# daxmawal/StarPU-Inference-Server

Measured on AMD Instinct MI355X. Metric: inferences/sec + p50 latency, ResNet-18 bs=1 & BERT-base seq=128, 1/2/4/8 GPU, higher is better.
Workload: dtype fp16m; 1 GPU; ResNet-18 bs=8 fp16, single MI355X HIP codelet (conv-as-implicit-GEMM MFMA); batch_per_task=8, workers_per_gpu=4, parallelism=replicas x1 (request sharding, no collective)

## Files before the change

starpu-inference-server_amd/csrc/conv_wres.hip:

```cpp
#include "lds_dma.hpp"
#include "spi_kernels.hpp"

#include <algorithm>
#include <cstdlib>
#include <stdexcept>
#include <type_traits>

namespace spi {
namespace {

constexpr int kRowB = 128;
constexpr int kWImg = 64 * kRowB;
constexpr int kWBytes = 9 * kWImg;
constexpr int kHaloPix = 256;
constexpr int kHBuf = kHaloPix * kRowB;
constexpr int kLds = kHBuf + kWBytes;
constexpr int BM = 128, BN = 64, NT = 256;
constexpr int kWPieces = kWBytes / 1024 / 4;
constexpr int kHPieces = kHBuf / 1024 / 4;

struct WresArgs {
  const _Float16* x;
  const char* w;
  const float* bias;
  const _Float16* res;
  _Float16* y;
  const char* zeros;
  int H, W;
  int th;
  int bands_per_img, bands;
};

#ifdef SPI_WRES_STAMPS
__device__ unsigned long long g_wres_stamps[4096 * 10];
#define WRES_STAMP(k)                                                                   \
  do {                                                                                  \
    __builtin_amdgcn_sched_barrier(0);                                                  \
    if (tid == 0 && blockIdx.x < 4096) g_wres_stamps[blockIdx.x * 10 + (k)] = __builtin_amdgcn_s_memtime(); \
    __builtin_amdgcn_sched_barrier(0);                                                  \
  } while (0)
#else
#define WRES_STAMP(k) \
  do {                \
  } while (0)
#endif

template <bool HAS_RES, bool RELU>
__global__ __launch_bounds__(NT, 1) void conv3x3_c64_wres(WresArgs a) {
  constexpr int kW0 = kHBuf;
  __shared__ __attribute__((aligned(16))) char lds[kLds];
  const int tid = threadIdx.x, lane = tid & 63, wave = __builtin_amdgcn_readfirstlane(tid >> 6);
  int wg = blockIdx.x;
  {
    const int nwg = gridDim.x, q = nwg >> 3, r = nwg & 7, x = wg & 7, l = wg >> 3;
    if (nwg >= 16) wg = (x < r ? x * (q + 1) : r * (q + 1) + (x - r) * q) + l;
  }
  const int band = wg;
  if (band >= a.bands) return;
  const int Wp = a.W + 2;
  const int hp = (a.th + 2) * Wp;
#ifdef SPI_WRES_STAMPS
  if (tid == 0 && blockIdx.x < 4096) g_wres_stamps[blockIdx.x * 10 + 9] = __builtin_amdgcn_s_memrealtime();
#endif
  WRES_STAMP(0);

  const char* wimg = a.w + (size_t)64 * (9 * kRowB);
  auto issue_w = [&] {
#pragma unroll
    for (int i = 0; i < kWPieces; ++i) {
      const int q = i * 4 + wave;
      glds16(wimg + q * 1024 + lane * 16, lds + kW0 + q * 1024);
    }
  };

  int h_hy[kHPieces], h_off[kHPieces];
  bool h_ok[kHPieces];
#pragma unroll
  for (int i = 0; i < kHPieces; ++i) {
    const int p = ((wave * kHPieces + i) << 3) + (lane >> 3);
    const int c = (lane & 7) ^ (p & 7);
    const int hy = p / Wp, hx = p - hy * Wp;
    h_hy[i] = hy;
    h_ok[i] = p < hp && (unsigned)(hx - 1) < (unsigned)a.W;
    h_off[i] = ((hy - 1) * a.W + (hx - 1)) * 64 + c * 8;
  }
  auto issue_halo = [&] {
    const int img = band / a.bands_per_img, oy0 = (band - img * a.bands_per_img) * a.th;
    const _Float16* base = a.x + ((size_t)img * a.H + oy0) * a.W * 64;
    char* dst = lds;
#pragma unroll
    for (int i = 0; i < kHPieces; ++i) {
      const int iy = oy0 - 1 + h_hy[i];
      const bool ok = h_ok[i] && (unsigned)iy < (unsigned)a.H;
      const char* src = ok ? reinterpret_cast<const char*>(base + h_off[i]) : a.zeros;
      glds16(src, dst + (wave * kHPieces + i) * 1024);
    }
  };

  const int fr = lane & 15, fq = lane >> 4, wm = wave >> 1, wn = wave & 1;
  int aoff[9][2][4];
#pragma unroll
  for (int i = 0; i < 4; ++i) {
    const int r = wm * 64 + i * 16 + fr;
    const int ty = r / a.W, tx = r - ty * a.W;
    const int p0 = ty < a.th ? ty * Wp + tx : 0;
#pragma unroll
    for (int tap = 0; tap < 9; ++tap)
#pragma unroll
      for (int kk = 0; kk < 2; ++kk) {
        const int p = p0 + (tap / 3) * Wp + tap % 3;
        aoff[tap][kk][i] = p * kRowB + (((kk * 4 + fq) ^ (p & 7)) << 4);
      }
  }
  int boff[2][2];
#pragma unroll
  for (int kk = 0; kk < 2; ++kk)
#pragma unroll
    for (int jj = 0; jj < 2; ++jj) {
      const int n = wn * 32 + jj * 16 + fr;
      boff[kk][jj] = kW0 + n * kRowB + (((kk * 4 + fq) ^ (n & 7)) << 4);
    }

  constexpr int E_G = BN / 8, E_RSTEP = NT / E_G, E_ITEMS = BM / E_RSTEP;
  const int e_nb8 = (tid % E_G) * 8, e_r0 = tid / E_G;
  int e_rel[E_ITEMS], e_ty[E_ITEMS];
#pragma unroll
  for (int it = 0; it < E_ITEMS; ++it) {
    const int row = e_r0 + it * E_RSTEP;
    const int ty = row / a.W, tx = row - ty * a.W;
    e_ty[it] = ty < a.th ? ty : 1 << 30;
    e_rel[it] = ty * a.W + tx;
  }

  issue_halo();
  issue_w();
  {
    [[maybe_unused]] constexpr int sk = 1;
    dma_wait_barrier<2 * 8>();
    WRES_STAMP(sk);
    const char* Hs = lds;

    floatx4 acc[4][2];
#pragma unroll
    for (int i = 0; i < 4; ++i)
#pragma unroll
      for (int jj = 0; jj < 2; ++jj) acc[i][jj] = floatx4{0.f, 0.f, 0.f, 0.f};
    half8 fa[2][4], fb[2][2];
    auto load = [&](int t, int s) {
      const int tap = t >> 1, kk = t & 1;
#pragma unroll
      for (int i = 0; i < 4; ++i) fa[s][i] = *reinterpret_cast<const half8*>(Hs + aoff[tap][kk][i]);
#pragma unroll
      for (int jj = 0; jj < 2; ++jj)
        fb[s][jj] = *reinterpret_cast<const half8*>(lds + boff[kk][jj] + tap * kWImg);
    };
    load(0, 0);
    static_for<0, 18>([&](auto tc) {
      constexpr int t = decltype(tc)::value;
      if constexpr (t + 1 < 18) {
        if constexpr ((t + 1) % 2 == 0) {
          constexpr int T = (t + 1) / 2;
          dma_wait_barrier<2 * (8 - T)>();
        }
        load(t + 1, (t + 1) & 1);
      }
      __builtin_amdgcn_sched_barrier(0);
#pragma unroll
      for (int i = 0; i < 4; ++i)
#pragma unroll
        for (int jj = 0; jj < 2; ++jj)
          acc[i][jj] = __builtin_amdgcn_mfma_f32_16x16x32_f16(fa[t & 1][i], fb[t & 1][jj], acc[i][jj], 0, 0, 0);
      __builtin_amdgcn_sched_barrier(0);
    });
    WRES_STAMP(sk + 1);

    const int img = band / a.bands_per_img, oy0 = (band - img * a.bands_per_img) * a.th;
    const int rows_left = a.H - oy0;
    const size_t mbase = ((size_t)img * a.H + oy0) * a.W;
    const floatx4 b0 = *reinterpret_cast<const floatx4*>(a.bias + e_nb8);
    const floatx4 b1 = *reinterpret_cast<const floatx4*>(a.bias + e_nb8 + 4);
    half8 rv[E_ITEMS];
    if constexpr (HAS_RES) {
#pragma unroll
      for (int it = 0; it < E_ITEMS; ++it) {
        const size_t mm = mbase + (e_ty[it] < rows_left ? e_rel[it] : 0);
        rv[it] = *reinterpret_cast<const half8*>(a.res + mm * 64 + e_nb8);
      }
    }
    lds_barrier();
#ifdef SPI_WRES_STAMPS_EPI
    if (sk == 1) WRES_STAMP(4);
#endif
    float* T = reinterpret_cast<float*>(lds);
#pragma unroll
    for (int i = 0; i < 4; ++i)
#pragma unroll
      for (int jj = 0; jj < 2; ++jj)
#pragma unroll
        for (int r = 0; r < 4; ++r) {
          const int row = wm * 64 + i * 16 + fq * 4 + r;
          const int col = (wn * 32 + jj * 16 + fr) ^ (fq << 4);
          T[row * BN + col] = acc[i][jj][r];
        }
#ifdef SPI_WRES_STAMPS_EPI
    if (sk == 1) WRES_STAMP(5);
#endif
    lds_barrier();
#ifdef SPI_WRES_STAMPS_EPI
    if (sk == 1) WRES_STAMP(6);
#endif
    half8 hv[E_ITEMS];
#pragma unroll
    for (int it = 0; it < E_ITEMS; ++it) {
      const int row = e_r0 + it * E_RSTEP;
      const float* src = T + row * BN + (e_nb8 ^ (((row >> 2) & 3) << 4));
      const floatx4 x0 = *reinterpret_cast<const floatx4*>(src);
      const floatx4 x1 = *reinterpret_cast<const floatx4*>(src + 4);
#pragma unroll
      for (int e = 0; e < 8; ++e) {
        float v = (e < 4 ? x0[e] + b0[e] : x1[e - 4] + b1[e - 4]);
        if constexpr (HAS_RES) v += static_cast<float>(rv[it][e]);
        if constexpr (RELU) v = v > 0.f ? v : 0.f;
        hv[it][e] = static_cast<_Float16>(v);
      }
    }
#pragma unroll
    for (int it = 0; it < E_ITEMS; ++it) {
#if defined(SPI_WRES_DIAG) && SPI_WRES_DIAG == 1
      asm volatile("" ::"v"(hv[it]));
#else
      if (e_ty[it] < rows_left) *reinterpret_cast<half8*>(a.y + (mbase + e_rel[it]) * 64 + e_nb8) = hv[it];
#endif
    }
    WRES_STAMP(sk + 2);
  }
  WRES_STAMP(7);
#ifdef SPI_WRES_STAMPS
  if (tid == 0 && blockIdx.x < 4096) g_wres_stamps[blockIdx.x * 10 + 8] = __builtin_amdgcn_s_memrealtime();
#endif
}

int env_int(const char* name, int dflt) {
  const char* e = std::getenv(name);
  return e && *e ? std::atoi(e) : dflt;
}

int& wres_on() {
  static int on = env_int("SPI_CONV_WRES", 1);
  return on;
}

}

void conv_wres_reload_env() { wres_on() = env_int("SPI_CONV_WRES", 1); }

#ifdef SPI_WRES_STAMPS
extern "C" int spi_debug_wres_stamps(unsigned long long* host, size_t n) {
  return hipMemcpyFromSymbol(host, HIP_SYMBOL(g_wres_stamps), n * sizeof(unsigned long long)) == hipSuccess ? 0 : 1;
}
#endif

static int wres_rows(int H, int W) {
  int th = std::min(H, BM / std::max(1, W));
  while (th > 0 && (th + 2) * (W + 2) > kHaloPix) --th;
  return th;
}

constexpr int kWresMaxTiles = 128;

bool conv_wres_eligible(const GemmDesc& d, Prec prec, const GemmPtrs& p) {
  const int on = wres_on();
  if (on == 1 && (d.M + 127) / 128 >= kWresMaxTiles) return false;
  const auto al16 = [](const void* q) { return (reinterpret_cast<uintptr_t>(q) & 15) == 0; };
  return on && prec == Prec::F16 && d.conv && d.KH == 3 && d.KW == 3 && d.stride == 1 && d.pad == 1 &&
         d.Cin == 64 && d.N == 64 && d.K == 576 && d.Kpad == 576 && d.krep == 1 && d.OH == d.H && d.OW == d.W &&
         !d.a_split && !d.out_split && !d.out_f32 && !d.res_f32 && !d.pool_rows && d.ldc == 64 &&
         (!p.res || d.ldr == 64) && d.act != Act::Gelu && wres_rows(d.H, d.W) >= 1 && al16(p.A) && al16(p.W) &&
         al16(p.C) && (!p.res || al16(p.res)) && (!p.bias || al16(p.bias)) && p.zeros && d.w_image;
}

void conv_wres(const GemmDesc& d, const GemmPtrs& p, hipStream_t s) {
  WresArgs a{};
  a.x = static_cast<const _Float16*>(p.A);
  a.w = static_cast<const char*>(p.W);
  a.bias = p.bias ? p.bias : static_cast<const float*>(p.zeros);
  a.res = static_cast<const _Float16*>(p.res);
  a.y = static_cast<_Float16*>(p.C);
  a.zeros = static_cast<const char*>(p.zeros);
  a.H = d.H;
  a.W = d.W;
  a.th = wres_rows(d.H, d.W);
  if (a.th < 1) throw std::invalid_argument("conv_wres: map too wide for the halo buffer");
  a.bands_per_img = (d.H + a.th - 1) / a.th;
  const int imgs = d.M / (d.OH * d.OW);
  a.bands = imgs * a.bands_per_img;
  const bool relu = d.act == Act::Relu;
  const dim3 grid(a.bands);
  if (a.res && relu)
    SPI_LAUNCH((conv3x3_c64_wres<true, true>), grid, dim3(NT), 0, s, a);
  else if (a.res)
    SPI_LAUNCH((conv3x3_c64_wres<true, false>), grid, dim3(NT), 0, s, a);
  else if (relu)
    SPI_LAUNCH((conv3x3_c64_wres<false, true>), grid, dim3(NT), 0, s, a);
  else
    SPI_LAUNCH((conv3x3_c64_wres<false, false>), grid, dim3(NT), 0, s, a);
}

}
```

Baseline: 116,400 inferences/s.

## Keep conv weights in registers per wave and drop weight LDS staging

Each wave now owns 16 output channels and holds its full 3x3x64 weight slice in registers, loaded directly from global memory. The kernel no longer stages weights through LDS, so LDS use shrinks to the halo buffer and launch bounds allow two workgroups per CU. A-operand addressing is computed incrementally, small integer divisions become float-reciprocal multiplies, and MFMA issue is interleaved with LDS reads through sched_group_barrier. This removes weight DMA and B-operand LDS reads. In exchange it costs more VGPRs for 18 weight fragments and 8 accumulators, and each wave now reads A fragments for all 128 rows.

```diff
diff --git a/starpu-inference-server_amd/csrc/conv_wres.hip b/starpu-inference-server_amd/csrc/conv_wres.hip
--- a/starpu-inference-server_amd/csrc/conv_wres.hip
+++ b/starpu-inference-server_amd/csrc/conv_wres.hip
@@ -10,13 +10,12 @@
 namespace {
 
 constexpr int kRowB = 128;
-constexpr int kWImg = 64 * kRowB;
-constexpr int kWBytes = 9 * kWImg;
+constexpr int kWRowB = 9 * kRowB;
 constexpr int kHaloPix = 256;
 constexpr int kHBuf = kHaloPix * kRowB;
-constexpr int kLds = kHBuf + kWBytes;
+constexpr int kLds = kHBuf;
 constexpr int BM = 128, BN = 64, NT = 256;
-constexpr int kWPieces = kWBytes / 1024 / 4;
+constexpr int kChunks = 18;
 constexpr int kHPieces = kHBuf / 1024 / 4;
 
 struct WresArgs {
@@ -46,8 +45,7 @@
 #endif
 
 template <bool HAS_RES, bool RELU>
-__global__ __launch_bounds__(NT, 1) void conv3x3_c64_wres(WresArgs a) {
-  constexpr int kW0 = kHBuf;
+__global__ __launch_bounds__(NT, 2) void conv3x3_c64_wres(WresArgs a) {
   __shared__ __attribute__((aligned(16))) char lds[kLds];
   const int tid = threadIdx.x, lane = tid & 63, wave = __builtin_amdgcn_readfirstlane(tid >> 6);
   int wg = blockIdx.x;
@@ -63,15 +61,8 @@
   if (tid == 0 && blockIdx.x < 4096) g_wres_stamps[blockIdx.x * 10 + 9] = __builtin_amdgcn_s_memrealtime();
 #endif
   WRES_STAMP(0);
-
-  const char* wimg = a.w + (size_t)64 * (9 * kRowB);
-  auto issue_w = [&] {
-#pragma unroll
-    for (int i = 0; i < kWPieces; ++i) {
-      const int q = i * 4 + wave;
-      glds16(wimg + q * 1024 + lane * 16, lds + kW0 + q * 1024);
-    }
-  };
+  const float invW = __builtin_amdgcn_rcpf((float)a.W), invWp = __builtin_amdgcn_rcpf((float)Wp);
+  const auto div_small = [](int n, float inv) { return (int)(((float)n + 0.5f) * inv); };
 
   int h_hy[kHPieces], h_off[kHPieces];
   bool h_ok[kHPieces];
@@ -79,7 +70,7 @@
   for (int i = 0; i < kHPieces; ++i) {
     const int p = ((wave * kHPieces + i) << 3) + (lane >> 3);
     const int c = (lane & 7) ^ (p & 7);
-    const int hy = p / Wp, hx = p - hy * Wp;
+    const int hy = div_small(p, invWp), hx = p - hy * Wp;
     h_hy[i] = hy;
     h_ok[i] = p < hp && (unsigned)(hx - 1) < (unsigned)a.W;
     h_off[i] = ((hy - 1) * a.W + (hx - 1)) * 64 + c * 8;
@@ -97,29 +88,17 @@
     }
   };
 
-  const int fr = lane & 15, fq = lane >> 4, wm = wave >> 1, wn = wave & 1;
-  int aoff[9][2][4];
-#pragma unroll
-  for (int i = 0; i < 4; ++i) {
-    const int r = wm * 64 + i * 16 + fr;
-    const int ty = r / a.W, tx = r - ty * a.W;
-    const int p0 = ty < a.th ? ty * Wp + tx : 0;
-#pragma unroll
-    for (int tap = 0; tap < 9; ++tap)
-#pragma unroll
-      for (int kk = 0; kk < 2; ++kk) {
-        const int p = p0 + (tap / 3) * Wp + tap % 3;
-        aoff[tap][kk][i] = p * kRowB + (((kk * 4 + fq) ^ (p & 7)) << 4);
-      }
-  }
-  int boff[2][2];
-#pragma unroll
-  for (int kk = 0; kk < 2; ++kk)
-#pragma unroll
-    for (int jj = 0; jj < 2; ++jj) {
-      const int n = wn * 32 + jj * 16 + fr;
-      boff[kk][jj] = kW0 + n * kRowB + (((kk * 4 + fq) ^ (n & 7)) << 4);
-    }
+  constexpr int TI = BM / 16;
+  const int fr = lane & 15, fq = lane >> 4;
+  int p0[TI];
+#pragma unroll
+  for (int i = 0; i < TI; ++i) {
+    const int r = i * 16 + fr;
+    const int ty = div_small(r, invW), tx = r - ty * a.W;
+    p0[i] = ty < a.th ? (ty * Wp + tx) << 4 : 0;
+  }
+  const int fq16 = fq << 4;
+  const char* wrow = a.w + (wave * 16 + fr) * kWRowB + fq * 16;
 
   constexpr int E_G = BN / 8, E_RSTEP = NT / E_G, E_ITEMS = BM / E_RSTEP;
   const int e_nb8 = (tid % E_G) * 8, e_r0 = tid / E_G;
@@ -127,49 +106,58 @@
 #pragma unroll
   for (int it = 0; it < E_ITEMS; ++it) {
     const int row = e_r0 + it * E_RSTEP;
-    const int ty = row / a.W, tx = row - ty * a.W;
+    const int ty = div_small(row, invW), tx = row - ty * a.W;
     e_ty[it] = ty < a.th ? ty : 1 << 30;
     e_rel[it] = ty * a.W + tx;
   }
 
   issue_halo();
-  issue_w();
+  half8 wb[kChunks];
+#pragma unroll
+  for (int t = 0; t < kChunks; ++t) {
+    wb[t] = *reinterpret_cast<const half8*>(wrow + t * 64);
+    __builtin_amdgcn_sched_barrier(0);
+  }
   {
     [[maybe_unused]] constexpr int sk = 1;
-    dma_wait_barrier<2 * 8>();
+    __builtin_amdgcn_sched_barrier(0);
+    dma_wait_barrier<kChunks>();
     WRES_STAMP(sk);
     const char* Hs = lds;
 
-    floatx4 acc[4][2];
-#pragma unroll
-    for (int i = 0; i < 4; ++i)
-#pragma unroll
-      for (int jj = 0; jj < 2; ++jj) acc[i][jj] = floatx4{0.f, 0.f, 0.f, 0.f};
-    half8 fa[2][4], fb[2][2];
+    floatx4 acc[TI];
+#pragma unroll
+    for (int i = 0; i < TI; ++i) acc[i] = floatx4{0.f, 0.f, 0.f, 0.f};
+    half8 fa[2][TI];
+    int ad[TI];
     auto load = [&](int t, int s) {
       const int tap = t >> 1, kk = t & 1;
-#pragma unroll
-      for (int i = 0; i < 4; ++i) fa[s][i] = *reinterpret_cast<const half8*>(Hs + aoff[tap][kk][i]);
-#pragma unroll
-      for (int jj = 0; jj < 2; ++jj)
-        fb[s][jj] = *reinterpret_cast<const half8*>(lds + boff[kk][jj] + tap * kWImg);
+      const int toff16 = ((tap / 3) * Wp + tap % 3) << 4;
+#pragma unroll
+      for (int i = 0; i < TI; ++i) {
+        if (kk == 0) {
+          const int p16 = p0[i] + toff16;
+          ad[i] = (p16 << 3) | ((p16 ^ fq16) & 0x70);
+        } else {
+          ad[i] ^= 64;
+        }
+        fa[s][i] = *reinterpret_cast<const half8*>(Hs + ad[i]);
+      }
     };
     load(0, 0);
-    static_for<0, 18>([&](auto tc) {
+    __builtin_amdgcn_sched_barrier(0);
+    static_for<0, kChunks>([&](auto tc) {
       constexpr int t = decltype(tc)::value;
-      if constexpr (t + 1 < 18) {
-        if constexpr ((t + 1) % 2 == 0) {
-          constexpr int T = (t + 1) / 2;
-          dma_wait_barrier<2 * (8 - T)>();
-        }
-        load(t + 1, (t + 1) & 1);
-      }
-      __builtin_amdgcn_sched_barrier(0);
-#pragma unroll
-      for (int i = 0; i < 4; ++i)
-#pragma unroll
-        for (int jj = 0; jj < 2; ++jj)
-          acc[i][jj] = __builtin_amdgcn_mfma_f32_16x16x32_f16(fa[t & 1][i], fb[t & 1][jj], acc[i][jj], 0, 0, 0);
+      if constexpr (t + 1 < kChunks) load(t + 1, (t + 1) & 1);
+#pragma unroll
+      for (int i = 0; i < TI; ++i)
+        acc[i] = __builtin_amdgcn_mfma_f32_16x16x32_f16(fa[t & 1][i], wb[t], acc[i], 0, 0, 0);
+#pragma unroll
+      for (int i = 0; i < TI; ++i) {
+        __builtin_amdgcn_sched_group_barrier(0x008, 1, 0);
+        __builtin_amdgcn_sched_group_barrier(0x002, (t + 1) & 1 ? 1 : 5, 0);
+        __builtin_amdgcn_sched_group_barrier(0x100, 1, 0);
+      }
       __builtin_amdgcn_sched_barrier(0);
     });
     WRES_STAMP(sk + 1);
@@ -193,15 +181,13 @@
 #endif
     float* T = reinterpret_cast<float*>(lds);
 #pragma unroll
-    for (int i = 0; i < 4; ++i)
-#pragma unroll
-      for (int jj = 0; jj < 2; ++jj)
-#pragma unroll
-        for (int r = 0; r < 4; ++r) {
-          const int row = wm * 64 + i * 16 + fq * 4 + r;
-          const int col = (wn * 32 + jj * 16 + fr) ^ (fq << 4);
-          T[row * BN + col] = acc[i][jj][r];
-        }
+    for (int i = 0; i < TI; ++i)
+#pragma unroll
+      for (int r = 0; r < 4; ++r) {
+        const int row = i * 16 + fq * 4 + r;
+        const int col = (wave * 16 + fr) ^ (fq << 4);
+        T[row * BN + col] = acc[i][r];
+      }
 #ifdef SPI_WRES_STAMPS_EPI
     if (sk == 1) WRES_STAMP(5);
 #endif
```

Measured after the change: 116,300 inferences/s. Within noise of the previous version (-0.0%).
